# lifeiteng/vall-e

Hardware: NVIDIA H100
Metric: audio tokens/sec (AR+NAR d=1024/12L) (higher is better)
Workload: dtype bf16

## Files before the change

### valle_b200/csrc/gemm_wgmma.cu

```cuda
#include <cuda.h>
#include <stdlib.h>

#include "common.cuh"
#include "kernels.cuh"
#include "sm90_ptx.cuh"

namespace vb {

namespace tc {

constexpr int BM = 128, BN = 128;
constexpr int kThreads = 384;
constexpr int kStages = 6;
constexpr int kABytes = BM * BK * 2;
constexpr int kBBytes = BN * BK * 2;
constexpr int kStageBytes = kABytes + kBBytes;
constexpr int kSmemBytes = kStages * kStageBytes + 1024  + 256 ;
static_assert(kSmemBytes <= 227 * 1024, "shared memory of one CTA");

template <int kEpi, typename TC>
__global__ void __launch_bounds__(kThreads, 1)
gemm_wgmma_kernel(const __grid_constant__ CUtensorMap tmap_a, const __grid_constant__ CUtensorMap tmap_b,
                  const float *__restrict__ bias, TC *__restrict__ C, int64_t ldc, int M, int K) {
  extern __shared__ uint8_t smem_raw[];
  uint8_t *tiles = reinterpret_cast<uint8_t *>((reinterpret_cast<uintptr_t>(smem_raw) + 1023) & ~(uintptr_t)1023);
  uint64_t *bars = reinterpret_cast<uint64_t *>(tiles + kStages * kStageBytes);
  uint64_t *full_bar = bars;
  uint64_t *empty_bar = bars + kStages;

  const int wg = threadIdx.x >> 7, t = threadIdx.x & 127;
  const int n_blk = blockIdx.x, m_blk = blockIdx.y;
  const int num_kb = K / BK;

  if (threadIdx.x == 0) {
    prefetch_tmap(&tmap_a);
    prefetch_tmap(&tmap_b);
    for (int i = 0; i < kStages; ++i) {
      mbar_init(&full_bar[i], 1);
      mbar_init(&empty_bar[i], 8);
    }
    asm volatile("fence.mbarrier_init.release.cluster;" ::: "memory");
  }
  __syncthreads();

  if (wg == 0) {
    if (t == 0) {
      int stage = 0;
      uint32_t phase = 0;
      for (int kb = 0; kb < num_kb; ++kb) {
        mbar_wait(&empty_bar[stage], phase ^ 1);
        uint8_t *a_dst = tiles + stage * kStageBytes;
        mbar_expect_tx(&full_bar[stage], kStageBytes);
        tma_load_2d(&tmap_a, &full_bar[stage], a_dst, kb * BK, m_blk * BM);
        tma_load_2d(&tmap_b, &full_bar[stage], a_dst + kABytes, kb * BK, n_blk * BN);
        if (++stage == kStages) {
          stage = 0;
          phase ^= 1;
        }
      }
    }
    return;
  }

  const int half = wg - 1;
  float acc[BN / 2];
  int stage = 0, prev = -1;
  uint32_t phase = 0;
  for (int kb = 0; kb < num_kb; ++kb) {
    mbar_wait(&full_bar[stage], phase);
    const uint32_t a_addr = smem_u32(tiles + stage * kStageBytes) + half * (64 * 128);
    const uint32_t b_addr = smem_u32(tiles + stage * kStageBytes) + kABytes;
    const uint64_t adesc = make_smem_desc(a_addr), bdesc = make_smem_desc(b_addr);
    wgmma_fence();
#pragma unroll
    for (int k = 0; k < BK / WGMMA_K; ++k) wgmma_m64n128k16(acc, adesc + (uint64_t)(k * 2), bdesc + (uint64_t)(k * 2), (kb | k) != 0);
    wgmma_commit();
    wgmma_wait<1>();
    if (prev >= 0 && (t & 31) == 0) mbar_arrive(&empty_bar[prev]);
    prev = stage;
    if (++stage == kStages) {
      stage = 0;
      phase ^= 1;
    }
  }
  wgmma_wait<0>();
  wgmma_fence_regs(acc);

  const int n0 = n_blk * BN;
#pragma unroll
  for (int i = 0; i < BN / 2; i += 2) {
    const int row = m_blk * BM + half * 64 + wg_row(t, i);
    const int col = n0 + wg_col(t, i);
    if (row >= M) continue;
    float v0 = acc[i], v1 = acc[i + 1];
    if (bias) {
      v0 += __ldg(bias + col);
      v1 += __ldg(bias + col + 1);
    }
    if constexpr (kEpi == VB_EPI_RELU) {
      v0 = fmaxf(v0, 0.f);
      v1 = fmaxf(v1, 0.f);
    }
    TC *dst = C + (int64_t)row * ldc + col;
    if constexpr (sizeof(TC) == 4) {
      float2 *d2 = reinterpret_cast<float2 *>(dst);
      if constexpr (kEpi == VB_EPI_RESIDUAL) {
        const float2 o = *d2;
        v0 = o.x + v0;
        v1 = o.y + v1;
      }
      *d2 = make_float2(v0, v1);
    } else {
      *reinterpret_cast<__nv_bfloat162 *>(dst) = __floats2bfloat162_rn(v0, v1);
    }
  }
}

template <int kEpi, typename TC>
static int launch_t(const CUtensorMap &ta, const CUtensorMap &tb, const float *bias, TC *C, int64_t ldc, int M,
                    int N, int K, cudaStream_t s) {
  auto kern = gemm_wgmma_kernel<kEpi, TC>;
  static PerDeviceOnce once;
  if (once.first()) VB_CUDA(cudaFuncSetAttribute(kern, cudaFuncAttributeMaxDynamicSharedMemorySize, kSmemBytes));
  const dim3 grid(N / BN, (M + BM - 1) / BM);
  kern<<<grid, kThreads, kSmemBytes, s>>>(ta, tb, bias, C, ldc, M, K);
  VB_LAUNCH_CHECK();
  return VB_OK;
}

}

bool wgmma_gemm_supported(int64_t M, int N, int K, int64_t lda, int64_t ldc) {
  return M >= 1 && (M + tc::BM - 1) / tc::BM <= 65535 && N % tc::BN == 0 && K % tc::BK == 0 && K > 0 &&
         lda % 8 == 0 && ldc % 8 == 0 && getenv("VB_DISABLE_WGMMA") == nullptr;
}

int launch_gemm_wgmma(const bf16 *A, int64_t lda, const bf16 *W, const float *bias, void *C, int c_dtype,
                      int64_t ldc, int64_t M, int N, int K, int epi, cudaStream_t s) {
  VB_CHECK_ARG((reinterpret_cast<uintptr_t>(A) & 15) == 0 && (reinterpret_cast<uintptr_t>(W) & 15) == 0 &&
                   (reinterpret_cast<uintptr_t>(C) & 15) == 0,
               "wgmma gemm: operands must be 16-byte aligned");
  CUtensorMap ta, tb;
  VB_TRY(tc::make_tmap(&ta, A, M, K, lda, tc::BM));
  VB_TRY(tc::make_tmap(&tb, W, N, K, K, tc::BN));
  const int m = (int)M;
  if (epi == VB_EPI_RESIDUAL) return tc::launch_t<VB_EPI_RESIDUAL, float>(ta, tb, bias, (float *)C, ldc, m, N, K, s);
  if (epi == VB_EPI_RELU) {
    if (c_dtype == VB_BF16) return tc::launch_t<VB_EPI_RELU, bf16>(ta, tb, bias, (bf16 *)C, ldc, m, N, K, s);
    return tc::launch_t<VB_EPI_RELU, float>(ta, tb, bias, (float *)C, ldc, m, N, K, s);
  }
  if (c_dtype == VB_BF16) return tc::launch_t<VB_EPI_NONE, bf16>(ta, tb, bias, (bf16 *)C, ldc, m, N, K, s);
  return tc::launch_t<VB_EPI_NONE, float>(ta, tb, bias, (float *)C, ldc, m, N, K, s);
}

}
```

### valle_b200/csrc/sm90_ptx.cuh

```cuda
#pragma once
#include <cuda.h>

#include <mutex>

#include "common.cuh"

namespace vb {
namespace tc {

constexpr int BK = 64;
constexpr int WGMMA_K = 16;

__device__ __forceinline__ uint32_t smem_u32(const void *p) {
  return static_cast<uint32_t>(__cvta_generic_to_shared(p));
}
__device__ __forceinline__ void mbar_init(uint64_t *bar, uint32_t count) {
  asm volatile("mbarrier.init.shared::cta.b64 [%0], %1;" ::"r"(smem_u32(bar)), "r"(count));
}
__device__ __forceinline__ void mbar_expect_tx(uint64_t *bar, uint32_t bytes) {
  asm volatile("mbarrier.arrive.expect_tx.shared::cta.b64 _, [%0], %1;" ::"r"(smem_u32(bar)), "r"(bytes)
               : "memory");
}
__device__ __forceinline__ void mbar_arrive(uint64_t *bar) {
  asm volatile("mbarrier.arrive.shared::cta.b64 _, [%0];" ::"r"(smem_u32(bar)) : "memory");
}
__device__ __forceinline__ uint32_t mbar_try_wait(uint64_t *bar, uint32_t parity) {
  uint32_t ok;
  asm volatile(
      "{\n"
      ".reg .pred p;\n"
      "mbarrier.try_wait.parity.shared::cta.b64 p, [%1], %2;\n"
      "selp.u32 %0, 1, 0, p;\n"
      "}\n"
      : "=r"(ok)
      : "r"(smem_u32(bar)), "r"(parity)
      : "memory");
  return ok;
}
__device__ __forceinline__ void mbar_wait(uint64_t *bar, uint32_t parity) {
  while (!mbar_try_wait(bar, parity)) {
  }
}
__device__ __forceinline__ void tma_load_2d(const CUtensorMap *map, uint64_t *bar, void *dst, int c0, int c1) {
  asm volatile(
      "cp.async.bulk.tensor.2d.shared::cluster.global.tile.mbarrier::complete_tx::bytes [%0], [%1, {%3, %4}], [%2];"
      ::"r"(smem_u32(dst)), "l"(map), "r"(smem_u32(bar)), "r"(c0), "r"(c1)
      : "memory");
}
__device__ __forceinline__ void prefetch_tmap(const CUtensorMap *map) {
  asm volatile("prefetch.tensormap [%0];" ::"l"(map) : "memory");
}
__device__ __forceinline__ void wgmma_fence() { asm volatile("wgmma.fence.sync.aligned;" ::: "memory"); }
__device__ __forceinline__ void wgmma_commit() { asm volatile("wgmma.commit_group.sync.aligned;" ::: "memory"); }
template <int N> __device__ __forceinline__ void wgmma_wait() {
  asm volatile("wgmma.wait_group.sync.aligned %0;" ::"n"(N) : "memory");
}
template <int R> __device__ __forceinline__ void wgmma_fence_regs(float (&d)[R]) {
#pragma unroll
  for (int i = 0; i < R; ++i) asm volatile("" : "+f"(d[i])::"memory");
}
__device__ __forceinline__ uint64_t make_smem_desc(uint32_t smem_addr) {
  uint64_t d = 0;
  d |= (uint64_t)((smem_addr & 0x3FFFF) >> 4);
  d |= (uint64_t)1 << 16;
  d |= (uint64_t)(1024 >> 4) << 32;
  d |= (uint64_t)1 << 62;
  return d;
}
__device__ __forceinline__ int wg_row(int t, int i) { return ((t >> 5) << 4) + ((t & 31) >> 2) + (((i >> 1) & 1) << 3); }
__device__ __forceinline__ int wg_col(int t, int i) { return ((i >> 2) << 3) + ((t & 3) << 1) + (i & 1); }

__device__ __forceinline__ void wgmma_m64n64k16(float (&d)[32], uint64_t adesc, uint64_t bdesc, uint32_t accumulate) {
  asm volatile(
      "{\n"
      ".reg .pred p;\n"
      "setp.ne.b32 p, %34, 0;\n"
      "wgmma.mma_async.sync.aligned.m64n64k16.f32.bf16.bf16 "
      "{%0, %1, %2, %3, %4, %5, %6, %7, %8, %9, %10, %11, %12, %13, %14, %15, %16, %17, %18, %19, %20, %21, %22, %23, %24, %25, %26, %27, %28, %29, %30, %31}, "
      "%32, %33, p, 1, 1, 0, 0;\n"
      "}\n"
      : "+f"(d[0]), "+f"(d[1]), "+f"(d[2]), "+f"(d[3]), "+f"(d[4]), "+f"(d[5]), "+f"(d[6]), "+f"(d[7]), "+f"(d[8]), "+f"(d[9]), "+f"(d[10]), "+f"(d[11]), "+f"(d[12]), "+f"(d[13]), "+f"(d[14]), "+f"(d[15]), "+f"(d[16]), "+f"(d[17]), "+f"(d[18]), "+f"(d[19]), "+f"(d[20]), "+f"(d[21]), "+f"(d[22]), "+f"(d[23]), "+f"(d[24]), "+f"(d[25]), "+f"(d[26]), "+f"(d[27]), "+f"(d[28]), "+f"(d[29]), "+f"(d[30]), "+f"(d[31])
      : "l"(adesc), "l"(bdesc), "r"(accumulate));
}

__device__ __forceinline__ void wgmma_m64n128k16(float (&d)[64], uint64_t adesc, uint64_t bdesc, uint32_t accumulate) {
  asm volatile(
      "{\n"
      ".reg .pred p;\n"
      "setp.ne.b32 p, %66, 0;\n"
      "wgmma.mma_async.sync.aligned.m64n128k16.f32.bf16.bf16 "
      "{%0, %1, %2, %3, %4, %5, %6, %7, %8, %9, %10, %11, %12, %13, %14, %15, %16, %17, %18, %19, %20, %21, %22, %23, %24, %25, %26, %27, %28, %29, %30, %31, %32, %33, %34, %35, %36, %37, %38, %39, %40, %41, %42, %43, %44, %45, %46, %47, %48, %49, %50, %51, %52, %53, %54, %55, %56, %57, %58, %59, %60, %61, %62, %63}, "
      "%64, %65, p, 1, 1, 0, 0;\n"
      "}\n"
      : "+f"(d[0]), "+f"(d[1]), "+f"(d[2]), "+f"(d[3]), "+f"(d[4]), "+f"(d[5]), "+f"(d[6]), "+f"(d[7]), "+f"(d[8]), "+f"(d[9]), "+f"(d[10]), "+f"(d[11]), "+f"(d[12]), "+f"(d[13]), "+f"(d[14]), "+f"(d[15]), "+f"(d[16]), "+f"(d[17]), "+f"(d[18]), "+f"(d[19]), "+f"(d[20]), "+f"(d[21]), "+f"(d[22]), "+f"(d[23]), "+f"(d[24]), "+f"(d[25]), "+f"(d[26]), "+f"(d[27]), "+f"(d[28]), "+f"(d[29]), "+f"(d[30]), "+f"(d[31]), "+f"(d[32]), "+f"(d[33]), "+f"(d[34]), "+f"(d[35]), "+f"(d[36]), "+f"(d[37]), "+f"(d[38]), "+f"(d[39]), "+f"(d[40]), "+f"(d[41]), "+f"(d[42]), "+f"(d[43]), "+f"(d[44]), "+f"(d[45]), "+f"(d[46]), "+f"(d[47]), "+f"(d[48]), "+f"(d[49]), "+f"(d[50]), "+f"(d[51]), "+f"(d[52]), "+f"(d[53]), "+f"(d[54]), "+f"(d[55]), "+f"(d[56]), "+f"(d[57]), "+f"(d[58]), "+f"(d[59]), "+f"(d[60]), "+f"(d[61]), "+f"(d[62]), "+f"(d[63])
      : "l"(adesc), "l"(bdesc), "r"(accumulate));
}

__device__ __forceinline__ void wgmma_m64n64k16_rs_tb(float (&d)[32], const uint32_t (&a)[4], uint64_t bdesc) {
  asm volatile(
      "{\n"
      ".reg .pred p;\n"
      "setp.ne.b32 p, %37, 0;\n"
      "wgmma.mma_async.sync.aligned.m64n64k16.f32.bf16.bf16 "
      "{%0, %1, %2, %3, %4, %5, %6, %7, %8, %9, %10, %11, %12, %13, %14, %15, %16, %17, %18, %19, %20, %21, %22, %23, %24, %25, %26, %27, %28, %29, %30, %31}, "
      "{%32, %33, %34, %35}, %36, p, 1, 1, 1;\n"
      "}\n"
      : "+f"(d[0]), "+f"(d[1]), "+f"(d[2]), "+f"(d[3]), "+f"(d[4]), "+f"(d[5]), "+f"(d[6]), "+f"(d[7]), "+f"(d[8]), "+f"(d[9]), "+f"(d[10]), "+f"(d[11]), "+f"(d[12]), "+f"(d[13]), "+f"(d[14]), "+f"(d[15]), "+f"(d[16]), "+f"(d[17]), "+f"(d[18]), "+f"(d[19]), "+f"(d[20]), "+f"(d[21]), "+f"(d[22]), "+f"(d[23]), "+f"(d[24]), "+f"(d[25]), "+f"(d[26]), "+f"(d[27]), "+f"(d[28]), "+f"(d[29]), "+f"(d[30]), "+f"(d[31])
      : "r"(a[0]), "r"(a[1]), "r"(a[2]), "r"(a[3]), "l"(bdesc), "r"(1));
}

typedef CUresult (*EncodeTiledFn)(CUtensorMap *, CUtensorMapDataType, cuuint32_t, void *, const cuuint64_t *,
                                  const cuuint64_t *, const cuuint32_t *, const cuuint32_t *,
                                  CUtensorMapInterleave, CUtensorMapSwizzle, CUtensorMapL2promotion,
                                  CUtensorMapFloatOOBfill);

inline EncodeTiledFn get_encode() {
  static EncodeTiledFn fn = nullptr;
  static std::once_flag once;
  std::call_once(once, [] {
    void *p = nullptr;
    cudaDriverEntryPointQueryResult q;
    if (cudaGetDriverEntryPoint("cuTensorMapEncodeTiled", &p, cudaEnableDefault, &q) == cudaSuccess &&
        q == cudaDriverEntryPointSuccess)
      fn = reinterpret_cast<EncodeTiledFn>(p);
  });
  return fn;
}

inline int make_tmap_f32_dense(CUtensorMap *map, const void *ptr, int64_t rows, int64_t cols, int64_t ld, int box_rows,
                               int box_cols) {
  EncodeTiledFn enc = get_encode();
  if (!enc) {
    set_error("tensor map: cuTensorMapEncodeTiled entry point unavailable");
    return VB_ERR_CUDA;
  }
  cuuint64_t dims[2] = {(cuuint64_t)cols, (cuuint64_t)rows};
  cuuint64_t strides[1] = {(cuuint64_t)ld * 4};
  cuuint32_t box[2] = {(cuuint32_t)box_cols, (cuuint32_t)box_rows};
  cuuint32_t estr[2] = {1, 1};
  CUresult r = enc(map, CU_TENSOR_MAP_DATA_TYPE_FLOAT32, 2, const_cast<void *>(ptr), dims, strides, box, estr,
                   CU_TENSOR_MAP_INTERLEAVE_NONE, CU_TENSOR_MAP_SWIZZLE_NONE, CU_TENSOR_MAP_L2_PROMOTION_L2_256B,
                   CU_TENSOR_MAP_FLOAT_OOB_FILL_NONE);
  if (r != CUDA_SUCCESS) {
    set_error("tensor map: cuTensorMapEncodeTiled (fp32 dense) failed (%d) rows=%lld cols=%lld ld=%lld", (int)r,
              (long long)rows, (long long)cols, (long long)ld);
    return VB_ERR_CUDA;
  }
  return VB_OK;
}
inline int make_tmap(CUtensorMap *map, const void *ptr, int64_t rows, int K, int64_t ld, int box_rows) {
  EncodeTiledFn enc = get_encode();
  if (!enc) {
    set_error("wgmma gemm: cuTensorMapEncodeTiled entry point unavailable");
    return VB_ERR_CUDA;
  }
  cuuint64_t dims[2] = {(cuuint64_t)K, (cuuint64_t)rows};
  cuuint64_t strides[1] = {(cuuint64_t)ld * 2};
  cuuint32_t box[2] = {(cuuint32_t)BK, (cuuint32_t)box_rows};
  cuuint32_t estr[2] = {1, 1};
  CUresult r = enc(map, CU_TENSOR_MAP_DATA_TYPE_BFLOAT16, 2, const_cast<void *>(ptr), dims, strides, box, estr,
                   CU_TENSOR_MAP_INTERLEAVE_NONE, CU_TENSOR_MAP_SWIZZLE_128B, CU_TENSOR_MAP_L2_PROMOTION_L2_256B,
                   CU_TENSOR_MAP_FLOAT_OOB_FILL_NONE);
  if (r != CUDA_SUCCESS) {
    set_error("wgmma gemm: cuTensorMapEncodeTiled failed (%d) rows=%lld K=%d ld=%lld", (int)r, (long long)rows, K,
              (long long)ld);
    return VB_ERR_CUDA;
  }
  return VB_OK;
}

}
}
```

Measured before the change: 230,900.

## Make WGMMA GEMM persistent with ping-pong consumer warpgroups and register reallocation

The GEMM becomes persistent: the grid is capped at the SM count and each CTA walks tiles in a strided loop. The two consumer warpgroups now each compute a full 128x128 tile and alternate tiles, ordered by named barriers, so one group's epilogue overlaps the other's MMA main loop. setmaxnreg moves registers from the producer to the consumers, and the producer issues L2 bulk prefetches of the residual output rows. The residual epilogue also batches its loads before its stores. The aim is to hide epilogue and launch tail costs, at the price of higher register pressure and more complex barrier phase bookkeeping.

New measurement: 239,800 (median of 6 runs). +3.9%, better.

```diff
diff --git a/valle_b200/csrc/gemm_wgmma.cu b/valle_b200/csrc/gemm_wgmma.cu
--- a/valle_b200/csrc/gemm_wgmma.cu
+++ b/valle_b200/csrc/gemm_wgmma.cu
@@ -17,11 +17,64 @@
 constexpr int kStageBytes = kABytes + kBBytes;
 constexpr int kSmemBytes = kStages * kStageBytes + 1024  + 256 ;
 static_assert(kSmemBytes <= 227 * 1024, "shared memory of one CTA");
+constexpr int kProducerRegs = 40, kConsumerRegs = 232;
+
+template <int kEpi, typename TC>
+__device__ __forceinline__ void store_fragment(const float (&acc)[BN / 2], const float *__restrict__ bias,
+                                               TC *__restrict__ C, int64_t ldc, int row0, int n0, int M, int t) {
+  if constexpr (kEpi == VB_EPI_RESIDUAL) {
+    static_assert(sizeof(TC) == 4, "the residual stream is fp32");
+    constexpr int kBatch = 32;
+#pragma unroll
+    for (int j = 0; j < BN / 2; j += kBatch) {
+      float2 o[kBatch / 2];
+#pragma unroll
+      for (int q = 0; q < kBatch / 2; ++q) {
+        const int i = j + 2 * q, row = row0 + wg_row(t, i);
+        o[q] = row < M ? *reinterpret_cast<const float2 *>(C + (int64_t)row * ldc + n0 + wg_col(t, i))
+                       : make_float2(0.f, 0.f);
+      }
+#pragma unroll
+      for (int q = 0; q < kBatch / 2; ++q) {
+        const int i = j + 2 * q, row = row0 + wg_row(t, i), col = n0 + wg_col(t, i);
+        if (row >= M) continue;
+        float v0 = acc[i], v1 = acc[i + 1];
+        if (bias) {
+          v0 += __ldg(bias + col);
+          v1 += __ldg(bias + col + 1);
+        }
+        *reinterpret_cast<float2 *>(C + (int64_t)row * ldc + col) = make_float2(o[q].x + v0, o[q].y + v1);
+      }
+    }
+  } else {
+#pragma unroll
+    for (int i = 0; i < BN / 2; i += 2) {
+      const int row = row0 + wg_row(t, i), col = n0 + wg_col(t, i);
+      if (row >= M) continue;
+      float v0 = acc[i], v1 = acc[i + 1];
+      if (bias) {
+        v0 += __ldg(bias + col);
+        v1 += __ldg(bias + col + 1);
+      }
+      if constexpr (kEpi == VB_EPI_RELU) {
+        v0 = fmaxf(v0, 0.f);
+        v1 = fmaxf(v1, 0.f);
+      }
+      TC *dst = C + (int64_t)row * ldc + col;
+      if constexpr (sizeof(TC) == 4) {
+        *reinterpret_cast<float2 *>(dst) = make_float2(v0, v1);
+      } else {
+        *reinterpret_cast<__nv_bfloat162 *>(dst) = __floats2bfloat162_rn(v0, v1);
+      }
+    }
+  }
+}
 
 template <int kEpi, typename TC>
 __global__ void __launch_bounds__(kThreads, 1)
 gemm_wgmma_kernel(const __grid_constant__ CUtensorMap tmap_a, const __grid_constant__ CUtensorMap tmap_b,
-                  const float *__restrict__ bias, TC *__restrict__ C, int64_t ldc, int M, int K) {
+                  const float *__restrict__ bias, TC *__restrict__ C, int64_t ldc, int M, int n_blks, int num_tiles,
+                  int K) {
   extern __shared__ uint8_t smem_raw[];
   uint8_t *tiles = reinterpret_cast<uint8_t *>((reinterpret_cast<uintptr_t>(smem_raw) + 1023) & ~(uintptr_t)1023);
   uint64_t *bars = reinterpret_cast<uint64_t *>(tiles + kStages * kStageBytes);
@@ -29,7 +82,6 @@
   uint64_t *empty_bar = bars + kStages;
 
   const int wg = threadIdx.x >> 7, t = threadIdx.x & 127;
-  const int n_blk = blockIdx.x, m_blk = blockIdx.y;
   const int num_kb = K / BK;
 
   if (threadIdx.x == 0) {
@@ -37,82 +89,79 @@
     prefetch_tmap(&tmap_b);
     for (int i = 0; i < kStages; ++i) {
       mbar_init(&full_bar[i], 1);
-      mbar_init(&empty_bar[i], 8);
+      mbar_init(&empty_bar[i], 4);
     }
     asm volatile("fence.mbarrier_init.release.cluster;" ::: "memory");
   }
   __syncthreads();
 
   if (wg == 0) {
+    setmaxnreg_dec<kProducerRegs>();
     if (t == 0) {
       int stage = 0;
       uint32_t phase = 0;
-      for (int kb = 0; kb < num_kb; ++kb) {
-        mbar_wait(&empty_bar[stage], phase ^ 1);
-        uint8_t *a_dst = tiles + stage * kStageBytes;
-        mbar_expect_tx(&full_bar[stage], kStageBytes);
-        tma_load_2d(&tmap_a, &full_bar[stage], a_dst, kb * BK, m_blk * BM);
-        tma_load_2d(&tmap_b, &full_bar[stage], a_dst + kABytes, kb * BK, n_blk * BN);
-        if (++stage == kStages) {
-          stage = 0;
-          phase ^= 1;
+      for (int tile = blockIdx.x; tile < num_tiles; tile += gridDim.x) {
+        const int m_blk = tile / n_blks, n_blk = tile - m_blk * n_blks;
+        if constexpr (kEpi == VB_EPI_RESIDUAL) {
+          const int rows = min(BM, M - m_blk * BM);
+          for (int r = 0; r < rows; ++r)
+            prefetch_l2_bulk(C + (int64_t)(m_blk * BM + r) * ldc + n_blk * BN, BN * sizeof(TC));
         }
+        for (int kb = 0; kb < num_kb; ++kb) {
+          mbar_wait(&empty_bar[stage], phase ^ 1);
+          uint8_t *a_dst = tiles + stage * kStageBytes;
+          mbar_expect_tx(&full_bar[stage], kStageBytes);
+          tma_load_2d(&tmap_a, &full_bar[stage], a_dst, kb * BK, m_blk * BM);
+          tma_load_2d(&tmap_b, &full_bar[stage], a_dst + kABytes, kb * BK, n_blk * BN);
+          if (++stage == kStages) {
+            stage = 0;
+            phase ^= 1;
+          }
+        }
       }
     }
     return;
   }
 
-  const int half = wg - 1;
-  float acc[BN / 2];
-  int stage = 0, prev = -1;
-  uint32_t phase = 0;
-  for (int kb = 0; kb < num_kb; ++kb) {
-    mbar_wait(&full_bar[stage], phase);
-    const uint32_t a_addr = smem_u32(tiles + stage * kStageBytes) + half * (64 * 128);
-    const uint32_t b_addr = smem_u32(tiles + stage * kStageBytes) + kABytes;
-    const uint64_t adesc = make_smem_desc(a_addr), bdesc = make_smem_desc(b_addr);
-    wgmma_fence();
-#pragma unroll
-    for (int k = 0; k < BK / WGMMA_K; ++k) wgmma_m64n128k16(acc, adesc + (uint64_t)(k * 2), bdesc + (uint64_t)(k * 2), (kb | k) != 0);
-    wgmma_commit();
-    wgmma_wait<1>();
-    if (prev >= 0 && (t & 31) == 0) mbar_arrive(&empty_bar[prev]);
-    prev = stage;
-    if (++stage == kStages) {
-      stage = 0;
-      phase ^= 1;
-    }
-  }
-  wgmma_wait<0>();
-  wgmma_fence_regs(acc);
-
-  const int n0 = n_blk * BN;
-#pragma unroll
-  for (int i = 0; i < BN / 2; i += 2) {
-    const int row = m_blk * BM + half * 64 + wg_row(t, i);
-    const int col = n0 + wg_col(t, i);
-    if (row >= M) continue;
-    float v0 = acc[i], v1 = acc[i + 1];
-    if (bias) {
-      v0 += __ldg(bias + col);
-      v1 += __ldg(bias + col + 1);
-    }
-    if constexpr (kEpi == VB_EPI_RELU) {
-      v0 = fmaxf(v0, 0.f);
-      v1 = fmaxf(v1, 0.f);
-    }
-    TC *dst = C + (int64_t)row * ldc + col;
-    if constexpr (sizeof(TC) == 4) {
-      float2 *d2 = reinterpret_cast<float2 *>(dst);
-      if constexpr (kEpi == VB_EPI_RESIDUAL) {
-        const float2 o = *d2;
-        v0 = o.x + v0;
-        v1 = o.y + v1;
-      }
-      *d2 = make_float2(v0, v1);
-    } else {
-      *reinterpret_cast<__nv_bfloat162 *>(dst) = __floats2bfloat162_rn(v0, v1);
-    }
+  setmaxnreg_inc<kConsumerRegs>();
+  const int c = wg - 1;
+  float acc0[BN / 2], acc1[BN / 2];
+  for (int j = c;; j += 2) {
+    const int tile = blockIdx.x + j * gridDim.x;
+    if (tile >= num_tiles) break;
+    const int m_blk = tile / n_blks, n_blk = tile - m_blk * n_blks;
+    const uint32_t it0 = (uint32_t)j * (uint32_t)num_kb;
+    int stage = (int)(it0 % kStages), prev = -1;
+    uint32_t phase = (it0 / kStages) & 1;
+    if (j > 0) asm volatile("bar.sync %0, 256;" ::"r"(1 + c) : "memory");
+    for (int kb = 0; kb < num_kb; ++kb) {
+      mbar_wait(&full_bar[stage], phase);
+      const uint32_t a_addr = smem_u32(tiles + stage * kStageBytes);
+      const uint64_t adesc0 = make_smem_desc(a_addr), adesc1 = make_smem_desc(a_addr + 64 * 128);
+      const uint64_t bdesc = make_smem_desc(a_addr + kABytes);
+      wgmma_fence();
+#pragma unroll
+      for (int k = 0; k < BK / WGMMA_K; ++k) {
+        wgmma_m64n128k16(acc0, adesc0 + (uint64_t)(k * 2), bdesc + (uint64_t)(k * 2), (kb | k) != 0);
+        wgmma_m64n128k16(acc1, adesc1 + (uint64_t)(k * 2), bdesc + (uint64_t)(k * 2), (kb | k) != 0);
+      }
+      wgmma_commit();
+      wgmma_wait<1>();
+      if (prev >= 0 && (t & 31) == 0) mbar_arrive(&empty_bar[prev]);
+      prev = stage;
+      if (++stage == kStages) {
+        stage = 0;
+        phase ^= 1;
+      }
+    }
+    if (tile + (int)gridDim.x < num_tiles) asm volatile("bar.arrive %0, 256;" ::"r"(2 - c) : "memory");
+    wgmma_wait<0>();
+    wgmma_fence_regs(acc0);
+    wgmma_fence_regs(acc1);
+    if ((t & 31) == 0) mbar_arrive(&empty_bar[prev]);
+
+    store_fragment<kEpi>(acc0, bias, C, ldc, m_blk * BM, n_blk * BN, M, t);
+    store_fragment<kEpi>(acc1, bias, C, ldc, m_blk * BM + 64, n_blk * BN, M, t);
   }
 }
 
@@ -122,8 +171,8 @@
   auto kern = gemm_wgmma_kernel<kEpi, TC>;
   static PerDeviceOnce once;
   if (once.first()) VB_CUDA(cudaFuncSetAttribute(kern, cudaFuncAttributeMaxDynamicSharedMemorySize, kSmemBytes));
-  const dim3 grid(N / BN, (M + BM - 1) / BM);
-  kern<<<grid, kThreads, kSmemBytes, s>>>(ta, tb, bias, C, ldc, M, K);
+  const int n_blks = N / BN, num_tiles = n_blks * ((M + BM - 1) / BM);
+  kern<<<min(sm_count(), num_tiles), kThreads, kSmemBytes, s>>>(ta, tb, bias, C, ldc, M, n_blks, num_tiles, K);
   VB_LAUNCH_CHECK();
   return VB_OK;
 }
diff --git a/valle_b200/csrc/sm90_ptx.cuh b/valle_b200/csrc/sm90_ptx.cuh
--- a/valle_b200/csrc/sm90_ptx.cuh
+++ b/valle_b200/csrc/sm90_ptx.cuh
@@ -49,6 +49,15 @@
 }
 __device__ __forceinline__ void prefetch_tmap(const CUtensorMap *map) {
   asm volatile("prefetch.tensormap [%0];" ::"l"(map) : "memory");
+}
+__device__ __forceinline__ void prefetch_l2_bulk(const void *p, uint32_t bytes) {
+  asm volatile("cp.async.bulk.prefetch.L2.global [%0], %1;" ::"l"(p), "r"(bytes) : "memory");
+}
+template <int R> __device__ __forceinline__ void setmaxnreg_inc() {
+  asm volatile("setmaxnreg.inc.sync.aligned.u32 %0;" ::"n"(R));
+}
+template <int R> __device__ __forceinline__ void setmaxnreg_dec() {
+  asm volatile("setmaxnreg.dec.sync.aligned.u32 %0;" ::"n"(R));
 }
 __device__ __forceinline__ void wgmma_fence() { asm volatile("wgmma.fence.sync.aligned;" ::: "memory"); }
 __device__ __forceinline__ void wgmma_commit() { asm volatile("wgmma.commit_group.sync.aligned;" ::: "memory"); }
```
